# bitmagier/q-learning

Measured on AMD Instinct MI355X. Metric: env-steps/sec + grad-updates/sec, Breakout 84×84×4, 1/2/4/8 MI355X, higher is better.
Workload: dtype fp32; 1 GPU; C3: 8192 Breakout envs per GPU, replay 1000000 per GPU in HBM (prefilled), Nature-DQN (3 conv + 2 dense) in fp32, B=1024, update every 128 env-steps per GPU (replay ratio 8 samples/env-step), epsilon-greedy acting; envs_per_gpu=8192, batch=1024, replay_capacity=1000000, update_after_actions=128, parallelism=single, rccl_world=1, global_batch_per_update=1024, env_dtype=fp32 physics, u8 frames, qnet_dtype=fp32 (exact-fp32 MFMA v_mfma_f32_16x16x4_f32)

## Files before the change

### q-learning_amd/csrc/qnet32.hip

```cpp
#include <hip/hip_ext.h>
#include <hip/hip_runtime.h>

#include <algorithm>
#include <cmath>
#include <cstdlib>
#include <map>
#include <tuple>
#include <vector>

#include "objects.h"
#include "profiler.h"
#include "qnet.h"
#include "qnet32_kernels.h"
#include "update32_dev.h"

namespace qlx {

using namespace q32;

struct F32Net {
  bool bg_rows = true;
  int c1_skip = 1;
  bool update_scheduled = false;
  bool dense_partials = false;
  float partials_scale = 1.0f;
  float *fa1 = nullptr, *fa2 = nullptr, *fa3 = nullptr, *fa4 = nullptr;
  float* fpart = nullptr;
  int *frl2 = nullptr, *frl3 = nullptr;
  unsigned long long* frcnt = nullptr;
  float* fbgc = nullptr;
  uint32_t* fsteps = nullptr;
  uint8_t* fneed = nullptr;
  int fneed_ld = 0;
  uint32_t* frows2 = nullptr;
  uint8_t* fbg2 = nullptr;
  uint32_t* frows3 = nullptr;
  uint8_t* fbg3 = nullptr;
  int fparity = 0;
  int frl_cap = 0;
  int fchunk = 0;
  DeviceBuffer<uint8_t> fgrad;
  int fgrad_batch = 0;
  float *fdz1 = nullptr, *fdz2 = nullptr, *fdz3 = nullptr, *fdz4 = nullptr;
  float *fslab1 = nullptr, *fslab2 = nullptr, *fslab3 = nullptr;
  float* fpb1 = nullptr;
  float* fpbg2 = nullptr;
  float* fs2 = nullptr;
  float* fpbg3 = nullptr;
  float* fs3 = nullptr;
};

constexpr int kHeadPitch = 514;
template <int MODE, int HS = 16>
__global__ __launch_bounds__(256) void k_head32(Fc2Args A) {
  __shared__ f32x4 part[4][16];
  __shared__ float gsh[16];
  __shared__ int ash[16];
  __shared__ __attribute__((aligned(16))) float xs[16 * kHeadPitch];
  __shared__ __attribute__((aligned(16))) float w4s[512 * 3];
  typedef float f32x2 __attribute__((ext_vector_type(2)));
  const int lane = threadIdx.x & 63, wave = threadIdx.x >> 6;
  const int s0 = blockIdx.x * HS;
  const int j = lane & 15, g = lane >> 4, n = lane & 15;
  const int b = s0 + j;
  const bool valid = j < HS && b < A.B;
  const bool tail = wave == 0 && g == 0 && valid;
  const int bt = tail ? b : 0;
  int t_act = 0;
  float t_y = 0.0f, t_w = 1.0f, t_r = 0.0f, t_qs[3] = {0.0f, 0.0f, 0.0f};
  bool t_done = false;
  if (tail) {
    if (MODE == 3) {
      t_act = A.actions[bt];
      t_y = A.y[bt];
      if (A.weights) t_w = A.weights[bt];
    } else if (MODE == 2) {
      t_r = A.rewards[bt];
      t_done = A.dones[bt] != 0;
      if (A.q_select)
        for (int r = 0; r < 3; ++r) t_qs[r] = A.q_select[bt * 3 + r];
    }
  }
  {
    f32x4 xr[8], wr[2];
#pragma unroll
    for (int r = 0; r < 8; ++r) {
      const int f = threadIdx.x + 256 * r, jj = f >> 7, k4 = f & 127;
      xr[r] = ld4(A.a4f + (size_t)(jj < HS && s0 + jj < A.B ? s0 + jj : s0) * 512 + 4 * k4);
    }
#pragma unroll
    for (int r = 0; r < 2; ++r) {
      const int f = threadIdx.x + 256 * r;
      if (f < 384) wr[r] = ld4(A.w4 + 4 * f);
    }
#pragma unroll
    for (int r = 0; r < 8; ++r) {
      const int f = threadIdx.x + 256 * r, jj = f >> 7, k4 = f & 127;
      f32x2* d = reinterpret_cast<f32x2*>(xs + jj * kHeadPitch + 4 * k4);
      d[0] = f32x2{xr[r][0], xr[r][1]};
      d[1] = f32x2{xr[r][2], xr[r][3]};
    }
#pragma unroll
// ... 426 lines not shown
  w.bg_rows = !(bg && bg[0] == '0');
  const char* sk = std::getenv("QLX_F32_C1_SKIP");
  w.c1_skip = (sk && sk[0] == '0') ? 0 : 1;
}

void f32_destroy(qlx_model* m) {
  delete m->fp32;
  m->fp32 = nullptr;
}

void f32_workspace(qlx_model* m, int B) {
  F32Net& w = *m->fp32;
  const int C = std::min(B, kF32FwdChunk);
  static_assert((uint64_t)kF32FwdChunk * 12800 * 4 < 0x80000000ull, "a forward chunk's a1 stays below 2^31 bytes");
  int nseg = 0;
  for (int v = 0; v < kNumVars; ++v) nseg += segs_of(v);
  const int frl_cap = C + kListSlots * (C / std::max(1, std::min(C, 2 * num_cus())) + 1) +
                      std::max(2 * num_cus(), C / kC1MaxIt + 1) + kListSlots;
  const int need_ld = (C + 63) / 64 * 64;
  ws_alloc(m, B, [&](Arena& a) {
    w.fa1 = a.take<float>((size_t)C * 12800); w.fa2 = a.take<float>((size_t)C * 5184); w.fa3 = a.take<float>((size_t)C * 3136);
    w.fa4 = a.take<float>((size_t)B * 512);
    w.fpart = a.take<float>(nseg);
    w.frl2 = a.take<int>((size_t)frl_cap * 81); w.frl3 = a.take<int>((size_t)frl_cap * 49);
    w.frcnt = a.take<unsigned long long>(2 * 2 * kListSlots * kCntStride);
    w.fbgc = a.take<float>(160);
    w.fsteps = a.take<uint32_t>((size_t)C * 4);
    w.fneed = a.take<uint8_t>((size_t)100 * need_ld);
    w.frows2 = a.take<uint32_t>((size_t)C * 4); w.fbg2 = a.take<uint8_t>((size_t)81 * need_ld);
    w.frows3 = a.take<uint32_t>((size_t)C * 4); w.fbg3 = a.take<uint8_t>((size_t)49 * need_ld);
  });
  QLX_HIP(hipMemset(w.frcnt, 0, 2 * 2 * kListSlots * kCntStride * 8));
  w.fneed_ld = need_ld;
  w.frl_cap = frl_cap;
  w.fparity = 0;
  w.fchunk = C;
}

static void f32_grad_workspace(qlx_model* m, int B) {
  F32Net& w = *m->fp32;
  if (B <= w.fgrad_batch) return;
  QLX_HIP(hipStreamSynchronize(m->stream));
  w.fgrad.release();
  w.fgrad_batch = 0;
  auto layout = [&](Arena& a) {
    w.fdz1 = a.take<float>((size_t)B * 12800); w.fdz2 = a.take<float>((size_t)B * 5184); w.fdz3 = a.take<float>((size_t)B * 3136);
    w.fdz4 = a.take<float>((size_t)B * 512);
    w.fslab1 = a.take<float>((size_t)((B + kSC1 - 1) / kSC1) * 257 * 32);
    w.fslab2 = a.take<float>((size_t)((B + kSC2 - 1) / kSC2) * 513 * 64);
    w.fslab3 = a.take<float>((size_t)((B + kSC3 - 1) / kSC3) * 577 * 64);
    w.fpb1 = a.take<float>((size_t)((B + 15) / 16) * 400 * 32);
    w.fpbg2 = a.take<float>((size_t)((B + 15) / 16) * 81 * 64); w.fs2 = a.take<float>((size_t)((B + 15) / 16) * 64);
    w.fpbg3 = a.take<float>((size_t)((B + 15) / 16) * 49 * 64); w.fs3 = a.take<float>((size_t)((B + 15) / 16) * 64);
  };
  Arena size;
  layout(size);
  w.fgrad.alloc(size.off);
  Arena a{(uintptr_t)w.fgrad.get()};
  layout(a);
  w.fgrad_batch = B;
}

template <class P>
static void launch(qlx_model* m, const P& p, const char* scope, double work, hipStream_t s) {
  hipEvent_t ea = nullptr, eb = nullptr;
  if (m->prof) m->prof->ext(scope, work, &ea, &eb);
  hipExtLaunchKernelGGL(k_gemm32<P>, dim3(p.g.blocks()), dim3(threads_of<P>()), gemm_lds_bytes<P>(), s, ea, eb, 0u, p);
  QLX_HIP(hipGetLastError());
  debug_sync(s, scope);
}

template <class P1, class P2, class S, class T = NoSide>
static void launch_pair(qlx_model* m, const P1& p1, const P2& p2, const S& side, const char* scope, double work, hipStream_t s,
                        const T& tail = T{}) {
  const size_t lds = std::max({gemm_lds_bytes<P1>(), gemm_lds_bytes<P2>(), S::LDS, T::LDS});
  hipEvent_t ea = nullptr, eb = nullptr;
  if (m->prof) m->prof->ext(scope, work, &ea, &eb);
  hipExtLaunchKernelGGL((k_gemm32_pair<P1, P2, S, T>), dim3(side.blocks() + p1.g.blocks() + p2.g.blocks() + tail.blocks()), dim3(256),
                        lds, s, ea, eb, 0u, p1, p2, side, tail);
  QLX_HIP(hipGetLastError());
  debug_sync(s, scope);
}

static int num_cus() {
  static int n = 0;
  if (!n) {
    const char* e = std::getenv("QLX_NUM_CUS");
    if (e && atoi(e) > 0) {
      n = atoi(e);
    } else {
      int dev = 0;
      QLX_HIP(hipGetDevice(&dev));
      QLX_HIP(hipDeviceGetAttribute(&n, hipDeviceAttributeMultiprocessorCount, dev));
    }
  }
  return n;
}

static Grid grid(int M, int BM, int N, int BN, int nz) { return Grid{(M + BM - 1) / BM, (N + BN - 1) / BN, nz}; }

static int c1_skip(const qlx_model* m) { return m->fp32->c1_skip; }

static int balanced_whole_tiles(int M) {
  const int ncu = num_cus(), t = M / 64, whole = t - t % ncu;
  if (whole < ncu || M - whole * 64 > 32 * ncu) return 0;
  return whole;
// ... 76 lines not shown
      if (big) {
        run(PConv2FwdL<64, 64, 2, 2>{}, PConv3FwdL<64, 64, 2, 2>{}, "f32_conv2_fwd_big", "f32_conv3_fwd_big");
        launch(m, PFc1FwdB{grid(n, PFc1FwdB::BM, 512, PFc1FwdB::BN, 1), w.fa3, p + var_offset(6), p + var_offset(7), w.fa4 + (size_t)c0 * 512, n}, "f32_fc1_fwd_big",
               2.0 * n * 3136 * 512, s);
      } else {
        run(PConv2FwdL<64, 64, 2, 2>{}, PConv3FwdL<32, 64, 2, 2>{}, "f32_conv2_fwd", "f32_conv3_fwd");
        launch(m, PFc1FwdS{grid(n, PFc1FwdS::BM, 512, PFc1FwdS::BN, 1), w.fa3, p + var_offset(6), p + var_offset(7), w.fa4 + (size_t)c0 * 512, n}, "f32_fc1_fwd",
               2.0 * n * 3136 * 512, s);
      }
    } else if (big) {
      launch(m, PConv2Fwd{grid(n * 81, 64, 64, 64, 1), w.fa1, p + var_offset(2), p + var_offset(3), w.fa2, n * 81}, "f32_conv2_fwd_big",
             2.0 * n * 81 * 64 * 512, s);
      launch(m, PConv3Fwd{grid(n * 49, 64, 64, 64, 1), w.fa2, p + var_offset(4), p + var_offset(5), w.fa3, n * 49}, "f32_conv3_fwd_big",
             2.0 * n * 49 * 64 * 576, s);
      launch(m, PFc1FwdB{grid(n, PFc1FwdB::BM, 512, PFc1FwdB::BN, 1), w.fa3, p + var_offset(6), p + var_offset(7), w.fa4 + (size_t)c0 * 512, n}, "f32_fc1_fwd_big",
             2.0 * n * 3136 * 512, s);
    } else {
      conv_fwd<PConv2Fwd, PConv2FwdR>(m, n * 81, w.fa1, p + var_offset(2), p + var_offset(3), w.fa2, "f32_conv2_fwd", 2.0 * n * 81 * 64 * 512, s,
                                      PConv2FwdS{grid(n * 81, 64, 64, 32, 1), w.fa1, p + var_offset(2), p + var_offset(3), w.fa2, n * 81});
      conv_fwd<PConv3Fwd, PConv3FwdR>(m, n * 49, w.fa2, p + var_offset(4), p + var_offset(5), w.fa3, "f32_conv3_fwd", 2.0 * n * 49 * 64 * 576, s,
                                      PConv3FwdS{grid(n * 49, 64, 64, 32, 1), w.fa2, p + var_offset(4), p + var_offset(5), w.fa3, n * 49});
      launch(m, PFc1FwdS{grid(n, PFc1FwdS::BM, 512, PFc1FwdS::BN, 1), w.fa3, p + var_offset(6), p + var_offset(7), w.fa4 + (size_t)c0 * 512, n}, "f32_fc1_fwd",
             2.0 * n * 3136 * 512, s);
    }
  }
}

void f32_head(int mode, const Fc2Args& a, int B, hipStream_t s) {
  constexpr int kHs3 = 4;
  const dim3 g((B + 15) / 16), blk(256);
  switch (mode) {
    case 0: hipLaunchKernelGGL(k_head32<0>, g, blk, 0, s, a); break;
    case 1: hipLaunchKernelGGL(k_head32<1>, g, blk, 0, s, a); break;
    case 2: hipLaunchKernelGGL(k_head32<2>, g, blk, 0, s, a); break;
    default: hipLaunchKernelGGL((k_head32<3, kHs3>), dim3((B + kHs3 - 1) / kHs3), blk, 0, s, a); break;
  }
  QLX_HIP(hipGetLastError());
  debug_sync(s, "k_head32");
}

Fc2Args f32_fc2_args(qlx_model* m, int B) {
  Fc2Args a = fc2_common(m, B);
  a.a4f = m->fp32->fa4;
  return a;
}

template <class Side>
static void f32_fc1_bwd(qlx_model* m, int B, const Side& S, hipStream_t s) {
  F32Net& w = *m->fp32;
  float* G = m->d_grads;
  const float* p = m->d_params;
  PFc1WgradS Pw{grid(3136, PFc1WgradS::BM, 512, PFc1WgradS::BN, 1), w.fa3, w.fdz4, G + var_offset(6), G + var_offset(7), B};
  PFc1DgradS Pd{grid(B, PFc1DgradS::BM, 3136, PFc1DgradS::BN, 1), w.fdz4, p + var_offset(6), w.fa3, w.fdz3, B};
  if (bg_rows(m)) {
    Pd.pbg = w.fpbg3;
    Pd.bg = w.fbg3;
    Pd.bg_ld = w.fneed_ld;
  }
  launch_pair(m, Pw, Pd, S, "f32_fc1_bwd", 2.0 * 2.0 * B * 512 * 3136, s);
}

void f32_backward_dense(qlx_model* m, int B, const uint8_t* actions, const float* y, float* loss_dev, hipStream_t s,
                        const float* weights, float* td_abs) {
  F32Net& w = *m->fp32;
  QLX_CHECK(B <= w.fchunk && B == m->last_batch, QLX_E_STATE, "f32 backward: batch must follow its forward");
  w.dense_partials = false;
  f32_grad_workspace(m, B);
  float* G = m->d_grads;
  float *gs = m->w.gs, *hs = m->w.hs;
  {
    ProfScope ps(m->prof, "f32_head", s);
    Fc2Args a = f32_fc2_args(m, B);
    a.actions = actions;
    a.y = y;
    a.gsample = gs;
    a.hsample = hs;
    a.weights = weights;
    a.td_abs = td_abs;
    a.dz4_out = w.fdz4;
    f32_head(3, a, B, s);
  }
  f32_fc1_bwd(m, B, SideFc2{w.fa4, actions, gs, hs, B, G + var_offset(8), G + var_offset(9), loss_dev}, s);
}

const float* f32_a4(qlx_model* m) { return m->fp32->fa4; }

float* f32_dz4_begin(qlx_model* m, int B) {
  F32Net& w = *m->fp32;
  QLX_CHECK(B <= w.fchunk && B == m->last_batch, QLX_E_STATE, "f32 backward: batch must follow its forward");
  w.dense_partials = false;
  f32_grad_workspace(m, B);
  return w.fdz4;
}

void f32_backward_dense_dz4(qlx_model* m, int B, const float* dq, hipStream_t s) {
  F32Net& w = *m->fp32;
  float* G = m->d_grads;
  f32_fc1_bwd(m, B, SideFc2Dq{w.fa4, nullptr, nullptr, nullptr, B, G + var_offset(8), G + var_offset(9), m->w.loss, dq}, s);
}

void f32_backward_dense_dq(qlx_model* m, int B, const float* dq, hipStream_t s) {
  float* dz4 = f32_dz4_begin(m, B);
  {
    ProfScope ps(m->prof, "f32_head_dq", s);
    hipLaunchKernelGGL(k_head32_dq, dim3((B + kHsDq - 1) / kHsDq), dim3(256), 0, s, f32_a4(m),
                       (const float*)(m->d_params + var_offset(8)), dq, B, dz4);
    QLX_HIP(hipGetLastError());
    debug_sync(s, "k_head32_dq");
  }
  f32_backward_dense_dz4(m, B, dq, s);
}

static void seg_tables(int* seg_first, int64_t* off) {
  int sf = 0;
  int64_t o = 0;
  for (int v = 0; v < kNumVars; ++v) {
    seg_first[v] = sf;
    off[v] = o;
    sf += segs_of(v);
    o += kVarSize[v];
  }
  seg_first[kNumVars] = sf;
  off[kNumVars] = o;
}

static NormArgs norm_args(qlx_model* m, float scale) {
  NormArgs A;
  A.g = m->d_grads;
  A.scale = scale;
  A.partial = m->fp32->fpart;
  seg_tables(A.seg_first, A.off);
  return A;
}

static Adam32Args adam_args(qlx_model* m, float scale) {
  const float tf = (float)(m->iterations + 1);
  const float b1p = std::pow(m->beta1, tf), b2p = std::pow(m->beta2, tf);
  Adam32Args a;
  a.w = m->d_params; a.m = m->d_m; a.v = m->d_v; a.g = m->d_grads; a.partial = m->fp32->fpart; a.norms = m->d_norms;
  seg_tables(a.seg_first, a.off);
  a.scale = scale;
  a.alpha = m->lr * std::sqrt(1.0f - b2p) / (1.0f - b1p);
  a.beta1 = m->beta1; a.beta2 = m->beta2; a.eps = m->eps; a.clipnorm = m->clipnorm;
  return a;
}

void f32_backward_conv(qlx_model* m, const uint8_t* const* table, int B, hipStream_t s, bool fuse_update, hipEvent_t dense_ready,
                       float dense_scale) {
  F32Net& w = *m->fp32;
  w.update_scheduled = fuse_update;
  QLX_CHECK(!(fuse_update && dense_ready), QLX_E_STATE, "dense partials: the scheduled update or the data-parallel form");
  const NormArgs N = norm_args(m, dense_ready ? dense_scale : 1.0f);
  const float* p = m->d_params;
  float* G = m->d_grads;
  const int z3 = (B + kSC3 - 1) / kSC3, z2 = (B + kSC2 - 1) / kSC2, z1 = (B + kSC1 - 1) / kSC1;
  {
    PConv3Wgrad Pw{grid(576, 64, 64, 64, z3), w.fa2, w.fdz3, w.fslab3, B, w.frows3};
    PConv3WgradD Pw_dense{grid(576, 64, 64, 64, z3), w.fa2, w.fdz3, w.fslab3, B};
    PConv3DgradP Pd{Grid{(B + PConv3DgradP::BM - 1) / PConv3DgradP::BM, 1, 81}, w.fdz3, p + var_offset(4), w.fa2, w.fdz2, B};
    if (bg_rows(m)) {
      Pd.pbg = w.fpbg2;
      Pd.bg2 = w.fbg2;
      Pd.bg2_ld = w.fneed_ld;
    }
    
    if (bg_rows(m)) launch_pair(m, Pw, Pd, SideBgSum<49>{w.fpbg3, w.fs3, z3}, "f32_conv3_bwd", 2.0 * 2.0 * B * 49 * 64 * 576, s);
    else launch_pair(m, Pw_dense, Pd, NoSide{}, "f32_conv3_bwd", 2.0 * 2.0 * B * 49 * 64 * 576, s);
  }
  {
    PConv2Wgrad Pw{grid(512, 64, 64, 64, z2), w.fa1, w.fdz2, w.fslab2, B, w.frows2};
    PConv2WgradD Pw_dense{grid(512, 64, 64, 64, z2), w.fa1, w.fdz2, w.fslab2, B};
    PConv2DgradP Pd{Grid{(B + 63) / 64, 2, 100}, w.fdz2, p + var_offset(2), w.fa1, w.fdz1, B, w.fpb1};
    if (c1_sparse_dz(m)) {
      Pd.need = w.fneed;
      Pd.need_ld = w.fneed_ld;
    }

    if (bg_rows(m)) launch_pair(m, Pw, Pd, SideBgSum<81>{w.fpbg2, w.fs2, z2}, "f32_conv2_bwd", 2.0 * 2.0 * B * 81 * 64 * 512, s);
    else launch_pair(m, Pw_dense, Pd, NoSide{}, "f32_conv2_bwd", 2.0 * 2.0 * B * 81 * 64 * 512, s);
  }
  {
    constexpr size_t lds = kC1WgradLds;
    hipEvent_t ea = nullptr, eb = nullptr;
    if (m->prof) m->prof->ext("f32_conv1_wgrad", 2.0 * B * 400 * 256 * 32, &ea, &eb);
    set_lds_limit((const void*)k_conv1_wgrad32, lds);
    const uint32_t* steps = c1_sparse_dz(m) ? w.fsteps : nullptr;
    hipExtLaunchKernelGGL(k_conv1_wgrad32, dim3(c1_wgrad_blocks(z1)), dim3(kC1WgradThreads), lds, s, ea, eb, 0u, table, w.fdz1, B, z1,
                          w.fslab1, c1_skip(m), steps, (const float*)w.fpb1);
    QLX_HIP(hipGetLastError());
    debug_sync(s, "k_conv1_wgrad32");
  }
  {
    ProfScope ps(m->prof, "f32_wgrad_reduce", s);
    WRed R;
    R.slab[0] = w.fslab3; R.nz[0] = z3; R.count[0] = 577 * 64; R.oc[0] = 64; R.gw[0] = G + var_offset(4); R.gb[0] = G + var_offset(5);
    R.slab[1] = w.fslab2; R.nz[1] = z2; R.count[1] = 513 * 64; R.oc[1] = 64; R.gw[1] = G + var_offset(2); R.gb[1] = G + var_offset(3);
    R.slab[2] = w.fslab1; R.nz[2] = z1; R.count[2] = 257 * 32; R.oc[2] = 32; R.gw[2] = G + var_offset(0); R.gb[2] = G + var_offset(1);
    R.sbg[0] = bg_rows(m) ? w.fs3 : nullptr;
    R.ubg[0] = w.fbgc + 32;
    R.sbg[1] = bg_rows(m) ? w.fs2 : nullptr;
    R.ubg[1] = w.fbgc;
    QLX_CHECK(std::max({z1, z2, z3}) <= kWGroup * kWGroupsMax, QLX_E_INVALID, "too many weight-gradient chunks");
    int nred = 0;
    for (int L = 0; L < 3; ++L) {
      R.wv[L] = wred_waves(R.nz[L]);
      const int per = 64 * (16 / R.wv[L]);
      R.nb[L] = (R.count[L] + per - 1) / per;
      nred += R.nb[L];
    }
    const bool dp_dense = dense_ready != nullptr;
    if (dp_dense) QLX_HIP(hipStreamWaitEvent(s, dense_ready, 0));
    const int dseg = w.update_scheduled || dp_dense ? N.seg_first[kNumVars] - N.seg_first[6] : 0;
    hipLaunchKernelGGL(k_wreduce32, dim3(nred + (dseg + 3) / 4), dim3(1024), 0, s, R, N, nred, N.seg_first[6], dseg);
    QLX_HIP(hipGetLastError());
    debug_sync(s, "k_wreduce32");
    if (dp_dense) {
      w.dense_partials = true;
      w.partials_scale = dense_scale;
    }
  }
}

void f32_gradient_replaced(qlx_model* m) { m->fp32->update_scheduled = m->fp32->dense_partials = false; }
// ... 117 lines not shown
```

### q-learning_amd/csrc/qnet32_kernels.h

```cpp
#pragma once
#include <hip/hip_runtime.h>

#include <cstdint>
#include <type_traits>

#include "qlx_internal.h"

namespace qlx {
namespace q32 {

typedef float f32x4 __attribute__((ext_vector_type(4)));

constexpr int BK = 32;
constexpr int kListSlots = 8;
constexpr int kCntStride = 16;

__host__ __device__ constexpr int kmaj_pad(int rows, int r) { return rows + ((r - rows % 64) % 64 + 64) % 64; }
__host__ __device__ constexpr int kmaj_pitch(int rows) {
  return kmaj_pad(rows, 48) < kmaj_pad(rows, 16) ? kmaj_pad(rows, 48) : kmaj_pad(rows, 16);
}
static_assert(kmaj_pitch(32) == 48 && kmaj_pitch(64) == 80 && kmaj_pitch(128) == 144, "KMAJ pitches");

template <int ROWS, bool KMAJ>
struct Opnd {
// ... 221 lines not shown
        if (O::F4 % T == 0 || tid + i * T < O::F4) rg[i] = buf_ld4(rs, vo[i], soff);
    } else {
#pragma unroll
      for (int i = 0; i < N; ++i)
        if (O::F4 % T == 0 || tid + i * T < O::F4) rg[i] = buf_ld4(rs, kk[i] < kvalid ? vo[i] : kOob, soff);
    }
  }
  __device__ void store(float* t, const Regs& rg) const {
#pragma unroll
    for (int i = 0; i < N; ++i) {
      const int idx = tid + i * T;
      if (O::F4 % T == 0 || idx < O::F4) {
        int r, k;
        O::coord(idx, r, k);
        O::put(t, r, k, rg[i]);
      }
    }
  }
};

template <class SA, class SB, uint32_t DA, uint32_t DB, bool KMASK = false>
struct PairStreams {
  SA a;
  SB b;
  int kmax;
  struct Regs {
    typename SA::Regs a;
    typename SB::Regs b;
  };
  __device__ void load(int s, Regs& x) const {
    const int kv = kmax - s * BK;
    a.load((uint32_t)s * DA, kv, x.a);
    b.load((uint32_t)s * DB, kv, x.b);
  }
  __device__ void store(float* as, float* bs, const Regs& x) const {
    a.store(as, x.a);
    b.store(bs, x.b);
  }
};

template <int T, bool PADS = true, int SHIFT = 0, uint32_t MASK = 0xFFFFFFFFu, uint32_t MUL = 1u>
struct TableK4Stream {
  static_assert(T == 256, "table gather stream: four waves");
  using O = Opnd<64, true>;
  static constexpr int N = 2;
  static constexpr uint32_t PAST = SHIFT == 0 && MASK == 0xFFFFFFFFu ? kOob : MASK * MUL;
  using Regs = f32x4[N];
  Rsrc rs;
  uint32_t vo;
  int tid, g, k0;
  const uint32_t* tbl;
  static constexpr int IMG = Opnd<64, true>::FLOATS, PITCH = Opnd<64, true>::PITCH;
  static_assert(PITCH == 80, "table stream: 16 pad columns per k-row");
  __host__ __device__ static int slot(int r) { return PADS ? (r >> 9) * IMG + ((r >> 4) & 31) * PITCH + 64 + (r & 15) : 4 * IMG + r; }
  __device__ void init(const void* base, uint32_t bytes, int tid_, uint32_t row_off) {
    rs = buf_rsrc(base, bytes);
    tid = tid_;
    g = (tid & 63) >> 4;
    k0 = q32_uniform(tid >> 6) * 4;
    vo = row_off;
  }
  __device__ void load(int kbase, Regs& rg) const {
#pragma unroll
    for (int i = 0; i < N; ++i) rg[i] = buf_ld4(rs, vo + ((tbl[slot(kbase + k0 + 16 * i + g)] >> SHIFT) & MASK) * MUL, 0u);
  }
  __device__ void store(float* t, const Regs& rg) const {
#pragma unroll
    for (int i = 0; i < N; ++i) O::put(t, (tid & 15) * 4, k0 + 16 * i + g, rg[i]);
  }
};

__host__ __device__ inline float ld_off(const float* base, uint32_t off) {
  return *reinterpret_cast<const float*>(reinterpret_cast<const char*>(base) + off);
}
__host__ __device__ inline void st_off(float* base, uint32_t off, float v) {
  *reinterpret_cast<float*>(reinterpret_cast<char*>(base) + off) = v;
}

template <class P, class = void>
struct ExtraLdsOf : std::integral_constant<size_t, 0> {};
template <class P>
struct ExtraLdsOf<P, std::void_t<decltype(P::EXTRA_LDS)>> : std::integral_constant<size_t, P::EXTRA_LDS> {};

template <class S, class = void>
struct HasPrepare : std::false_type {};
template <class S>
struct HasPrepare<S, std::void_t<decltype(std::declval<S&>().prepare((float*)nullptr, 0))>> : std::true_type {};

template <class P>
constexpr size_t gemm_lds_bytes() {
  return (size_t)KSplitOf<P>::value * 2 *
             (size_t)(Opnd<P::BM, P::A_KMAJ>::FLOATS + Opnd<P::BN, P::B_KMAJ>::FLOATS) * sizeof(float) +
         ExtraLdsOf<P>::value;
}

template <class P>
__device__ __forceinline__ void gemm_body(const P& p, int lb, float* lds) {
  constexpr int MF = 16;
  using OA = Opnd<P::BM, P::A_KMAJ>;
  using OB = Opnd<P::BN, P::B_KMAJ>;
  using Acc = f32x4;
  constexpr int TM = P::BM / (P::WM * MF), TN = P::BN / (P::WN * MF);
  static_assert(TM >= 1 && TN >= 1 && TM * P::WM * MF == P::BM && TN * P::WN * MF == P::BN, "tile shape");
  constexpr int G = KSplitOf<P>::value, Q = KSeqOf<P>::value;
  static_assert((G == 1 && Q <= 2) || (Q == 1 && !P::BIAS), "K split: two sequential chains, or wave groups without bias");
  static_assert(G == 1 || TM * TN * 4 * P::WM * P::WN * 64 <= 2 * (OA::FLOATS + OB::FLOATS), "K-split hand-off fits a group's LDS");
  constexpr int T = P::WM * P::WN * 64;
// ... 788 lines not shown
      d[r] = row + r < B && pr.m[r] > 0.0f ? v[r] : 0.0f;
      if (row + r < B && ((pr.nb >> (8 * r)) & 0xFFu) != 0u) st_off(dz1, (uint32_t)(row + r) * 51200u + po, d[r]);
    }
    if (pb) {
      const float s = pb_sum16(d);
      if ((row & 15) == 0 && row < B) pb[((size_t)(row >> 4) * 400 + ih * 20 + iw) * 32 + (col & 31)] = s;
    }
  }
  static constexpr int T = WM_ * WN_ * 64;
  struct Streams {
    AffineStream<BM_, false, T> a;
    AffineStream<BN_, false, T> b;
    Px q;
    struct Regs {
      typename AffineStream<BM_, false, T>::Regs a;
      typename AffineStream<BN_, false, T>::Regs b;
    };
    __device__ void load(int s, Regs& x) const {
      const int t = s >> 1, th = q.th0 + t / q.ntw, tw = q.tw0 + t % q.ntw, h = (s & 1) * 32;
      a.load((uint32_t)(((q.i - th) * 9 + q.j - tw) * 64 + h) * 4u, 0, x.a);
      b.load((uint32_t)((8 * th + 2 * tw) * 2048 + h) * 4u, 0, x.b);
    }
    __device__ void store(float* as, float* bs, const Regs& x) const {
      a.store(as, x.a);
      b.store(bs, x.b);
    }
  };
  __device__ Streams streams(int z, int row0, int col0, int tid) const {
    Streams st;
    st.q = px(z);
    const int nb = B;
    st.a.init(dz2, (uint32_t)B * 5184u * 4u, tid,
              [row0, nb](int r, int k) { return row0 + r < nb ? (uint32_t)((row0 + r) * 5184 + k) * 4u : kOob; });
    st.b.init(w1, 16u * 32u * 64u * 4u, tid, [col0](int r, int k) {
      const int col = col0 + r, cls = col >> 5;
      return (uint32_t)((((cls >> 1) * 4 + (cls & 1)) * 32 + (col & 31)) * 64 + k) * 4u;
    });
    return st;
  }
};

template <int H, int W, int C, int KS, int S, int OH, int OW, int OC, int SC, int BM_ = 64, int BN_ = 64, int WM_ = 2, int WN_ = 2,
          bool TPADS = true, bool CMP = false>
struct PConvWgrad {
  static constexpr int BM = BM_, BN = BN_, WM = WM_, WN = WN_;
  static constexpr bool LOAD_FENCE = false;
  static constexpr bool A_KMAJ = true, B_KMAJ = true, BIAS = true;
  static constexpr int MROWS = KS * KS * C, P = OH * OW, CHUNK = SC;
  Grid g;
  const float* in;
  const float* dz;
  float* slab;
  int B;
  const uint32_t* rows = nullptr;
  __host__ __device__ void decode(int lb, int& tm, int& tn, int& z) const { g.decode(lb, tm, tn, z); }
  __host__ __device__ int rows_in(int z) const {
    const int b0 = z * SC, b1 = b0 + SC < B ? b0 + SC : B;
    return (b1 - b0) * P;
  }
  static_assert(!CMP || (P <= 96 && SC * P <= 4096 && (size_t)SC * H * W * C * 4 <= 0xFFFFFu - 4 * KS * W * C),
                "compacted weight gradient: packed table entries");
  __host__ __device__ int kept_in(int z) const {
    int n = 0;
#if defined(__HIP_DEVICE_COMPILE__) && !defined(QLX_Q32_POLICIES_ONLY)
    if constexpr (CMP) {
      static_assert(SC * 4 == 64, "compacted weight gradient: a chunk's row words are one wave's lanes");
      const int wl = threadIdx.x & 63;
      const uint32_t wv = z * SC + (wl >> 2) < B && (wl & 3) != 3 ? rows[(size_t)z * SC * 4 + wl] : 0u;
      for (int l = 0; l < 64; ++l)
        if ((l & 3) != 3) n += __builtin_popcount(__builtin_amdgcn_readlane(wv, l));
      return n;
    }
#endif
    for (int bl = 0; bl < SC; ++bl) {
      const int b = z * SC + bl;
      if (b < B) n += __builtin_popcount(rows[(size_t)b * 4]) + __builtin_popcount(rows[(size_t)b * 4 + 1]) +
                      __builtin_popcount(rows[(size_t)b * 4 + 2]);
    }
    return n;
  }
  __host__ __device__ int nslabs(int z) const { return ((CMP ? kept_in(z) : rows_in(z)) + BK - 1) / BK; }
  __device__ void epi(int z, int row, int col, f32x4 v) const {
#pragma unroll
    for (int r = 0; r < 4; ++r) slab[((size_t)z * (MROWS + 1) + row + r) * OC + col] = v[r];
  }
  __device__ void epi_bias(int z, int col, float v) const { slab[((size_t)z * (MROWS + 1) + MROWS) * OC + col] = v; }
  static constexpr int T = WM_ * WN_ * 64;
  static constexpr int KMAX = (SC * P + BK - 1) / BK * BK;
  struct StreamsImpl {
    TableK4Stream<T, TPADS> a;
    AffineStream<BN_, true, T, true> b;
    int z, rows;
    struct Regs {
      typename TableK4Stream<T, TPADS>::Regs a;
      typename AffineStream<BN_, true, T, true>::Regs b;
    };
    __device__ void prepare(float* lds, int ns) {
      uint32_t* t = reinterpret_cast<uint32_t*>(lds);
      for (int r = a.tid; r < ns * BK; r += T) {
        uint32_t o = kOob;
        if (r < rows) {
          const int bl = r / P, pp = r - bl * P, oh = pp / OW, ow = pp - oh * OW;
          o = (uint32_t)((((z * SC + bl) * H + oh * S) * W + ow * S) * C) * 4u;
        }
        t[TableK4Stream<T, TPADS>::slot(r)] = o;
      }
      a.tbl = t;
    }
    __device__ void load(int s, Regs& x) const {
      const int kbase = s * BK;
      a.load(kbase, x.a);
      b.load((uint32_t)kbase * OC * 4u, rows - kbase, x.b);
    }
    __device__ void store(float* as, float* bs, const Regs& x) const {
      a.store(as, x.a);
      b.store(bs, x.b);
    }
  };
  using TA = TableK4Stream<T, TPADS, 0, 0xFFFFFu, 1u>;
  using TB = TableK4Stream<T, TPADS, 20, 0xFFFu, (uint32_t)OC * 4u>;
  struct StreamsCmp {
    TA a;
    TB b;
    int z;
    const uint32_t* rows;
    int B;
    struct Regs {
      typename TA::Regs a;
      typename TB::Regs b;
    };
    __device__ void prepare(float* lds, int ns) {
      uint32_t* t = reinterpret_cast<uint32_t*>(lds);
      int run = 0;
#ifndef QLX_Q32_POLICIES_ONLY
      static_assert(SC * 4 == 64, "compacted weight gradient: a chunk's row words are one wave's lanes");
      const int wl = a.tid & 63;
      const uint32_t wv = z * SC + (wl >> 2) < B ? rows[(size_t)z * SC * 4 + wl] : 0u;
#endif
      for (int bl = 0; bl < SC; ++bl) {
#ifdef QLX_Q32_POLICIES_ONLY
        const int b = z * SC + bl;
        const uint32_t w0 = b < B ? rows[(size_t)b * 4] : 0u, w1 = b < B ? rows[(size_t)b * 4 + 1] : 0u,
                       w2 = b < B ? rows[(size_t)b * 4 + 2] : 0u;
#else
        const uint32_t w0 = __builtin_amdgcn_readlane(wv, 4 * bl), w1 = __builtin_amdgcn_readlane(wv, 4 * bl + 1),
                       w2 = __builtin_amdgcn_readlane(wv, 4 * bl + 2);
#endif
        for (int pp = a.tid; pp < P; pp += T) {
          const uint32_t w = pp < 32 ? w0 : (pp < 64 ? w1 : w2), bit = 1u << (pp & 31);
          if (w & bit) {
            const int below = (pp >= 32 ? __builtin_popcount(w0) : 0) + (pp >= 64 ? __builtin_popcount(w1) : 0) +
                              __builtin_popcount(w & (bit - 1u));
            const int oh = pp / OW, ow = pp - oh * OW;
            const uint32_t ao = (uint32_t)(((bl * H + oh * S) * W + ow * S) * C) * 4u;
            t[TA::slot(run + below)] = ao | ((uint32_t)(bl * P + pp) << 20);
          }
        }
        run += __builtin_popcount(w0) + __builtin_popcount(w1) + __builtin_popcount(w2);
      }
      for (int r = run + a.tid; r < ns * BK; r += T) t[TA::slot(r)] = 0xFFFFFFFFu;
      a.tbl = t;
      b.tbl = t;
    }
    __device__ void load(int s, Regs& x) const {
      a.load(s * BK, x.a);
      b.load(s * BK, x.b);
    }
    __device__ void store(float* as, float* bs, const Regs& x) const {
      a.store(as, x.a);
      b.store(bs, x.b);
    }
  };
  static_assert(BM_ == 64 && WM_ * WN_ == 4, "weight gradient: the table stream stages 64-row tiles on four waves");
  using Streams = std::conditional_t<CMP, StreamsCmp, StreamsImpl>;
  static_assert(!TPADS || KMAX <= 4 * 32 * 16, "weight-gradient chunk: the offset table lives in the four images' pads");
  static_assert(!TPADS || BN_ == 64, "weight-gradient tiles with the table in the pads need BN = 64");
  static constexpr size_t EXTRA_LDS = !TPADS ? (size_t)KMAX * 4 : 0;
  __device__ Streams streams(int z, int row0, int col0, int tid) const {
    Streams st;
    st.z = z;
    const int m = row0 + (tid & 15) * 4, tap = m / C, c = m - tap * C, kh = tap / KS, kw = tap - kh * KS;
    if constexpr (CMP) {
      st.rows = rows;
      st.B = B;
      const int nb = B - z * SC < SC ? B - z * SC : SC;
      st.a.init(in + (size_t)z * SC * H * W * C, (uint32_t)nb * H * W * C * 4u, tid, (uint32_t)((kh * W + kw) * C + c) * 4u);
      st.b.init(dz + (size_t)z * SC * P * OC, (uint32_t)nb * P * OC * 4u, tid, (uint32_t)(col0 + (tid & 15) * 4) * 4u);
    } else {
      st.rows = rows_in(z);
      st.a.init(in, (uint32_t)B * H * W * C * 4u, tid, (uint32_t)((kh * W + kw) * C + c) * 4u);
      st.b.init(dz + (size_t)z * SC * P * OC, (uint32_t)st.rows * OC * 4u, tid,
                [col0](int r, int k) { return (uint32_t)(k * OC + col0 + r) * 4u; });
    }
    return st;
  }
};

constexpr int kSC1 = QLX_F32_WGRAD_CHUNK_CONV1, kSC2 = QLX_F32_WGRAD_CHUNK_CONV2, kSC3 = QLX_F32_WGRAD_CHUNK_CONV3;
using PConv3Wgrad = PConvWgrad<9, 9, 64, 3, 1, 7, 7, 64, kSC3, 64, 64, 1, 4, false, true>;
using PConv3WgradD = PConvWgrad<9, 9, 64, 3, 1, 7, 7, 64, kSC3, 64, 64, 1, 4, false>;
static_assert(kSC3 == 16, "conv3 weight-gradient chunks are the fc1 backward's 16-row fragments (pbg)");
using PConv2Wgrad = PConvWgrad<20, 20, 32, 4, 2, 9, 9, 64, kSC2, 64, 64, 1, 4, true, true>;
using PConv2WgradD = PConvWgrad<20, 20, 32, 4, 2, 9, 9, 64, kSC2, 64, 64, 1, 4>;
static_assert(kSC2 == 16, "conv2 weight-gradient chunks are the conv3 backward's 16-row fragments (pbg)");
using PConv3DgradP = PConv3DgradPx<64, 64, 2, 2>;
using PConv2DgradP = PConv2DgradPx<64, 64, 2, 2>;

template <bool DQ>
struct SideFc2T {
  static constexpr int BLOCKS = 33;
  __host__ __device__ int blocks() const { return BLOCKS; }
  static constexpr int HB = 512;
  static constexpr size_t LDS = (size_t)HB * 20 * sizeof(float);
  const float* a4;
  const uint8_t* act;
  const float* gs;
  const float* hs;
  int B;
  float* dw4;
  float* db4;
  float* loss;
  const float* dq = nullptr;
  __device__ void run(int t, float* lds) const {
    float* as = lds;
    float* ds = lds + HB * 16;
    const int tid = threadIdx.x, lane = tid & 63, g = lane >> 4, n = lane & 15;
    f32x4 acc = zero4();
    for (int b0 = 0; b0 < B; b0 += HB) {
      __syncthreads();
      if (t < 32) {
#pragma unroll
        for (int j = 0; j < HB * 4 / 256; ++j) {
          const int q = tid + 256 * j, bl = q >> 2, b = b0 + bl;
          f32x4 v = zero4();
          if (b < B) v = ld4(a4 + (size_t)b * 512 + t * 16 + (q & 3) * 4);
          *reinterpret_cast<f32x4*>(as + q * 4) = v;
        }
      }
#pragma unroll
      for (int j = 0; j < HB / 256; ++j) {
        const int bl = tid + 256 * j, b = b0 + bl;
        f32x4 v = zero4();
        if (b < B) {
          if constexpr (DQ) {
            v = f32x4{dq[(size_t)b * 3], dq[(size_t)b * 3 + 1], dq[(size_t)b * 3 + 2], 0.0f};
          } else {
            const int a = act[b];
            const float gv = gs[b];
            v = f32x4{a == 0 ? gv : 0.0f, a == 1 ? gv : 0.0f, a == 2 ? gv : 0.0f, hs[b]};
          }
        }
        *reinterpret_cast<f32x4*>(ds + bl * 4) = v;
      }
      __syncthreads();
      if (tid < 64) {
        const int S = (min(HB, B - b0) + 3) / 4;
#pragma unroll 8
// ... 481 lines not shown
```

Measured before the change: 333,800 env-steps/s.

## Prebuild compacted wgrad offset tables as side blocks during fc1 backward

Moves construction of the compacted row-offset tables for conv2/conv3 weight gradients out of every wgrad block's prepare phase. The tables are now built once per 16-sample chunk by extra side blocks launched alongside the fc1 backward pair, and stored in HBM. Wgrad blocks then copy the table into LDS with vector buffer loads and read the kept-row count from a stored word. This removes redundant per-tile table building and serial readlane loops, at the cost of extra workspace, an extra global round trip, and more work in the fc1 launch.

Result: no change. 335,800 env-steps/s, median of 6 (+0.6%).

```diff
diff --git a/q-learning_amd/csrc/qnet32.hip b/q-learning_amd/csrc/qnet32.hip
--- a/q-learning_amd/csrc/qnet32.hip
+++ b/q-learning_amd/csrc/qnet32.hip
@@ -48,6 +48,7 @@
   float* fs2 = nullptr;
   float* fpbg3 = nullptr;
   float* fs3 = nullptr;
+  uint32_t *ftbl2 = nullptr, *ftbl3 = nullptr;
 };
 
 constexpr int kHeadPitch = 514;
@@ -580,6 +581,8 @@
     w.fpb1 = a.take<float>((size_t)((B + 15) / 16) * 400 * 32);
     w.fpbg2 = a.take<float>((size_t)((B + 15) / 16) * 81 * 64); w.fs2 = a.take<float>((size_t)((B + 15) / 16) * 64);
     w.fpbg3 = a.take<float>((size_t)((B + 15) / 16) * 49 * 64); w.fs3 = a.take<float>((size_t)((B + 15) / 16) * 64);
+    w.ftbl2 = a.take<uint32_t>((size_t)((B + kSC2 - 1) / kSC2) * PConv2Wgrad::TSTRIDE);
+    w.ftbl3 = a.take<uint32_t>((size_t)((B + kSC3 - 1) / kSC3) * PConv3Wgrad::TSTRIDE);
   };
   Arena size;
   layout(size);
@@ -762,12 +765,15 @@
   const float* p = m->d_params;
   PFc1WgradS Pw{grid(3136, PFc1WgradS::BM, 512, PFc1WgradS::BN, 1), w.fa3, w.fdz4, G + var_offset(6), G + var_offset(7), B};
   PFc1DgradS Pd{grid(B, PFc1DgradS::BM, 3136, PFc1DgradS::BN, 1), w.fdz4, p + var_offset(6), w.fa3, w.fdz3, B};
+  ChunkTables tables;
   if (bg_rows(m)) {
     Pd.pbg = w.fpbg3;
     Pd.bg = w.fbg3;
     Pd.bg_ld = w.fneed_ld;
-  }
-  launch_pair(m, Pw, Pd, S, "f32_fc1_bwd", 2.0 * 2.0 * B * 512 * 3136, s);
+    static_assert(kSC2 == 16 && kSC3 == 16, "one table block per 16-sample chunk and layer");
+    tables = ChunkTables{w.frows3, w.ftbl3, w.frows2, w.ftbl2, B, (B + 15) / 16};
+  }
+  launch_pair(m, Pw, Pd, S, "f32_fc1_bwd", 2.0 * 2.0 * B * 512 * 3136, s, tables);
 }
 
 void f32_backward_dense(qlx_model* m, int B, const uint8_t* actions, const float* y, float* loss_dev, hipStream_t s,
@@ -865,7 +871,7 @@
   float* G = m->d_grads;
   const int z3 = (B + kSC3 - 1) / kSC3, z2 = (B + kSC2 - 1) / kSC2, z1 = (B + kSC1 - 1) / kSC1;
   {
-    PConv3Wgrad Pw{grid(576, 64, 64, 64, z3), w.fa2, w.fdz3, w.fslab3, B, w.frows3};
+    PConv3Wgrad Pw{grid(576, 64, 64, 64, z3), w.fa2, w.fdz3, w.fslab3, B, w.ftbl3};
     PConv3WgradD Pw_dense{grid(576, 64, 64, 64, z3), w.fa2, w.fdz3, w.fslab3, B};
     PConv3DgradP Pd{Grid{(B + PConv3DgradP::BM - 1) / PConv3DgradP::BM, 1, 81}, w.fdz3, p + var_offset(4), w.fa2, w.fdz2, B};
     if (bg_rows(m)) {
@@ -878,7 +884,7 @@
     else launch_pair(m, Pw_dense, Pd, NoSide{}, "f32_conv3_bwd", 2.0 * 2.0 * B * 49 * 64 * 576, s);
   }
   {
-    PConv2Wgrad Pw{grid(512, 64, 64, 64, z2), w.fa1, w.fdz2, w.fslab2, B, w.frows2};
+    PConv2Wgrad Pw{grid(512, 64, 64, 64, z2), w.fa1, w.fdz2, w.fslab2, B, w.ftbl2};
     PConv2WgradD Pw_dense{grid(512, 64, 64, 64, z2), w.fa1, w.fdz2, w.fslab2, B};
     PConv2DgradP Pd{Grid{(B + 63) / 64, 2, 100}, w.fdz2, p + var_offset(2), w.fa1, w.fdz1, B, w.fpb1};
     if (c1_sparse_dz(m)) {
diff --git a/q-learning_amd/csrc/qnet32_kernels.h b/q-learning_amd/csrc/qnet32_kernels.h
--- a/q-learning_amd/csrc/qnet32_kernels.h
+++ b/q-learning_amd/csrc/qnet32_kernels.h
@@ -297,7 +297,7 @@
   const uint32_t* tbl;
   static constexpr int IMG = Opnd<64, true>::FLOATS, PITCH = Opnd<64, true>::PITCH;
   static_assert(PITCH == 80, "table stream: 16 pad columns per k-row");
-  __host__ __device__ static int slot(int r) { return PADS ? (r >> 9) * IMG + ((r >> 4) & 31) * PITCH + 64 + (r & 15) : 4 * IMG + r; }
+  __host__ __device__ static constexpr int slot(int r) { return PADS ? (r >> 9) * IMG + ((r >> 4) & 31) * PITCH + 64 + (r & 15) : 4 * IMG + r; }
   __device__ void init(const void* base, uint32_t bytes, int tid_, uint32_t row_off) {
     rs = buf_rsrc(base, bytes);
     tid = tid_;
@@ -1192,7 +1192,7 @@
   const float* dz;
   float* slab;
   int B;
-  const uint32_t* rows = nullptr;
+  const uint32_t* tbl = nullptr;
   __host__ __device__ void decode(int lb, int& tm, int& tn, int& z) const { g.decode(lb, tm, tn, z); }
   __host__ __device__ int rows_in(int z) const {
     const int b0 = z * SC, b1 = b0 + SC < B ? b0 + SC : B;
@@ -1200,25 +1200,30 @@
   }
   static_assert(!CMP || (P <= 96 && SC * P <= 4096 && (size_t)SC * H * W * C * 4 <= 0xFFFFFu - 4 * KS * W * C),
                 "compacted weight gradient: packed table entries");
-  __host__ __device__ int kept_in(int z) const {
-    int n = 0;
-#if defined(__HIP_DEVICE_COMPILE__) && !defined(QLX_Q32_POLICIES_ONLY)
-    if constexpr (CMP) {
-      static_assert(SC * 4 == 64, "compacted weight gradient: a chunk's row words are one wave's lanes");
-      const int wl = threadIdx.x & 63;
-      const uint32_t wv = z * SC + (wl >> 2) < B && (wl & 3) != 3 ? rows[(size_t)z * SC * 4 + wl] : 0u;
-      for (int l = 0; l < 64; ++l)
-        if ((l & 3) != 3) n += __builtin_popcount(__builtin_amdgcn_readlane(wv, l));
-      return n;
-    }
-#endif
+  static constexpr int KMAX = (SC * P + BK - 1) / BK * BK;
+  static constexpr int TSTRIDE = KMAX + 4;
+  template <int NT, class WordFn>
+  __host__ __device__ static void build_table(WordFn word, uint32_t* out, int tid) {
+    int run = 0;
+#pragma unroll
     for (int bl = 0; bl < SC; ++bl) {
-      const int b = z * SC + bl;
-      if (b < B) n += __builtin_popcount(rows[(size_t)b * 4]) + __builtin_popcount(rows[(size_t)b * 4 + 1]) +
-                      __builtin_popcount(rows[(size_t)b * 4 + 2]);
-    }
-    return n;
-  }
+      const uint32_t w0 = word(bl, 0), w1 = word(bl, 1), w2 = word(bl, 2);
+      for (int pp = tid; pp < P; pp += NT) {
+        const uint32_t w = pp < 32 ? w0 : (pp < 64 ? w1 : w2), bit = 1u << (pp & 31);
+        if (w & bit) {
+          const int below = (pp >= 32 ? __builtin_popcount(w0) : 0) + (pp >= 64 ? __builtin_popcount(w1) : 0) +
+                            __builtin_popcount(w & (bit - 1u));
+          const int oh = pp / OW, ow = pp - oh * OW;
+          const uint32_t ao = (uint32_t)(((bl * H + oh * S) * W + ow * S) * C) * 4u;
+          out[run + below] = ao | ((uint32_t)(bl * P + pp) << 20);
+        }
+      }
+      run += __builtin_popcount(w0) + __builtin_popcount(w1) + __builtin_popcount(w2);
+    }
+    for (int r = run + tid; r < KMAX; r += NT) out[r] = 0xFFFFFFFFu;
+    if (tid == 0) out[KMAX] = (uint32_t)run;
+  }
+  __host__ __device__ int kept_in(int z) const { return (int)tbl[(size_t)z * TSTRIDE + KMAX]; }
   __host__ __device__ int nslabs(int z) const { return ((CMP ? kept_in(z) : rows_in(z)) + BK - 1) / BK; }
   __device__ void epi(int z, int row, int col, f32x4 v) const {
 #pragma unroll
@@ -1226,7 +1231,6 @@
   }
   __device__ void epi_bias(int z, int col, float v) const { slab[((size_t)z * (MROWS + 1) + MROWS) * OC + col] = v; }
   static constexpr int T = WM_ * WN_ * 64;
-  static constexpr int KMAX = (SC * P + BK - 1) / BK * BK;
   struct StreamsImpl {
     TableK4Stream<T, TPADS> a;
     AffineStream<BN_, true, T, true> b;
@@ -1262,43 +1266,15 @@
   struct StreamsCmp {
     TA a;
     TB b;
-    int z;
-    const uint32_t* rows;
-    int B;
+    Rsrc trs;
     struct Regs {
       typename TA::Regs a;
       typename TB::Regs b;
     };
     __device__ void prepare(float* lds, int ns) {
+      static_assert(TA::slot(4) == TA::slot(0) + 4 && TA::slot(12) % 4 == 0, "compacted weight gradient: four entries per LDS store");
       uint32_t* t = reinterpret_cast<uint32_t*>(lds);
-      int run = 0;
-#ifndef QLX_Q32_POLICIES_ONLY
-      static_assert(SC * 4 == 64, "compacted weight gradient: a chunk's row words are one wave's lanes");
-      const int wl = a.tid & 63;
-      const uint32_t wv = z * SC + (wl >> 2) < B ? rows[(size_t)z * SC * 4 + wl] : 0u;
-#endif
-      for (int bl = 0; bl < SC; ++bl) {
-#ifdef QLX_Q32_POLICIES_ONLY
-        const int b = z * SC + bl;
-        const uint32_t w0 = b < B ? rows[(size_t)b * 4] : 0u, w1 = b < B ? rows[(size_t)b * 4 + 1] : 0u,
-                       w2 = b < B ? rows[(size_t)b * 4 + 2] : 0u;
-#else
-        const uint32_t w0 = __builtin_amdgcn_readlane(wv, 4 * bl), w1 = __builtin_amdgcn_readlane(wv, 4 * bl + 1),
-                       w2 = __builtin_amdgcn_readlane(wv, 4 * bl + 2);
-#endif
-        for (int pp = a.tid; pp < P; pp += T) {
-          const uint32_t w = pp < 32 ? w0 : (pp < 64 ? w1 : w2), bit = 1u << (pp & 31);
-          if (w & bit) {
-            const int below = (pp >= 32 ? __builtin_popcount(w0) : 0) + (pp >= 64 ? __builtin_popcount(w1) : 0) +
-                              __builtin_popcount(w & (bit - 1u));
-            const int oh = pp / OW, ow = pp - oh * OW;
-            const uint32_t ao = (uint32_t)(((bl * H + oh * S) * W + ow * S) * C) * 4u;
-            t[TA::slot(run + below)] = ao | ((uint32_t)(bl * P + pp) << 20);
-          }
-        }
-        run += __builtin_popcount(w0) + __builtin_popcount(w1) + __builtin_popcount(w2);
-      }
-      for (int r = run + a.tid; r < ns * BK; r += T) t[TA::slot(r)] = 0xFFFFFFFFu;
+      for (int r = 4 * a.tid; r < ns * BK; r += 4 * T) *reinterpret_cast<f32x4*>(t + TA::slot(r)) = buf_ld4(trs, (uint32_t)r * 4u, 0u);
       a.tbl = t;
       b.tbl = t;
     }
@@ -1318,15 +1294,14 @@
   static constexpr size_t EXTRA_LDS = !TPADS ? (size_t)KMAX * 4 : 0;
   __device__ Streams streams(int z, int row0, int col0, int tid) const {
     Streams st;
-    st.z = z;
     const int m = row0 + (tid & 15) * 4, tap = m / C, c = m - tap * C, kh = tap / KS, kw = tap - kh * KS;
     if constexpr (CMP) {
-      st.rows = rows;
-      st.B = B;
+      st.trs = buf_rsrc(tbl + (size_t)z * TSTRIDE, (uint32_t)KMAX * 4u);
       const int nb = B - z * SC < SC ? B - z * SC : SC;
       st.a.init(in + (size_t)z * SC * H * W * C, (uint32_t)nb * H * W * C * 4u, tid, (uint32_t)((kh * W + kw) * C + c) * 4u);
       st.b.init(dz + (size_t)z * SC * P * OC, (uint32_t)nb * P * OC * 4u, tid, (uint32_t)(col0 + (tid & 15) * 4) * 4u);
     } else {
+      st.z = z;
       st.rows = rows_in(z);
       st.a.init(in, (uint32_t)B * H * W * C * 4u, tid, (uint32_t)((kh * W + kw) * C + c) * 4u);
       st.b.init(dz + (size_t)z * SC * P * OC, (uint32_t)st.rows * OC * 4u, tid,
@@ -1343,6 +1318,30 @@
 using PConv2Wgrad = PConvWgrad<20, 20, 32, 4, 2, 9, 9, 64, kSC2, 64, 64, 1, 4, true, true>;
 using PConv2WgradD = PConvWgrad<20, 20, 32, 4, 2, 9, 9, 64, kSC2, 64, 64, 1, 4>;
 static_assert(kSC2 == 16, "conv2 weight-gradient chunks are the conv3 backward's 16-row fragments (pbg)");
+
+struct ChunkTables {
+  static constexpr size_t LDS = 0;
+  const uint32_t* rows3 = nullptr;
+  uint32_t* tbl3 = nullptr;
+  const uint32_t* rows2 = nullptr;
+  uint32_t* tbl2 = nullptr;
+  int B = 0, nz = 0;
+  __host__ __device__ int blocks() const { return 2 * nz; }
+#ifndef QLX_Q32_POLICIES_ONLY
+  template <class PW>
+  __device__ void build(const uint32_t* rows, uint32_t* tbl, int z) const {
+    static_assert(PW::CHUNK * 4 == 64, "compacted weight gradient: a chunk's row words are one wave's lanes");
+    const int wl = threadIdx.x & 63;
+    const uint32_t wv = z * PW::CHUNK + (wl >> 2) < B ? rows[(size_t)z * 64 + wl] : 0u;
+    PW::template build_table<256>([wv](int bl, int i) { return (uint32_t)__builtin_amdgcn_readlane(wv, 4 * bl + i); },
+                                  tbl + (size_t)z * PW::TSTRIDE, (int)threadIdx.x);
+  }
+  __device__ void run(int blk, float*) const {
+    if (blk & 1) build<PConv2Wgrad>(rows2, tbl2, blk >> 1);
+    else build<PConv3Wgrad>(rows3, tbl3, blk >> 1);
+  }
+#endif
+};
 using PConv3DgradP = PConv3DgradPx<64, 64, 2, 2>;
 using PConv2DgradP = PConv2DgradPx<64, 64, 2, 2>;
 
```
